# ygtxr1997/MSML

Measured on AMD Instinct MI355X. Metric: images/sec (112x112) ires50-MSML+PartialFC training step, higher is better.
Workload: dtype bf16; 1 GPU; iresnet50-MSML (OSB r18 + FM x4) + 85742-id ArcFace PartialFC, 112x112, batch 256/GPU, fwd+bwd+clip+SGD; global_batch=256, parallelism=dp1+class-parallel head, launch=eager, weight gradients + OSB on side streams

## Files before the change

### include/msml_hip.h

```cpp
#ifndef MSML_HIP_H
#define MSML_HIP_H

#include <stddef.h>
#include <stdint.h>

#ifdef __cplusplus
extern "C" {
#endif

#define MSML_ABI_VERSION 1

enum { MSML_F32 = 0, MSML_BF16 = 1, MSML_BF16X3 = 2,
       MSML_F64 = 3 };

enum {
  MSML_OK = 0,
  MSML_ERR_SHAPE = -1,
  MSML_ERR_DTYPE = -2,
  MSML_ERR_LAUNCH = -3,
  MSML_ERR_UNSUPPORTED = -4,
  MSML_ERR_WORKSPACE = -5,
  MSML_ERR_CAPACITY = -6
};

// ... 216 lines not shown

int msml_deconv4_bwd_data(const void* dy, const void* wp0, const void* wp1, void* dx0, void* dx1, int N, int H,
                          void* stream);

int msml_conv2d_bnbwd_rows(int coutp, int N, int P, int Q);
int msml_conv2d_bnbwd(const void* in0, int c0p, const void* wp, int kop, void* out, int coutp,
                      int N, int H, int W, int P, int Q, int R, int S, int stride, int pad_h,
                      int pad_w, int transposed, const void* bn_x, const float* bn_scale,
                      const float* bn_shift, const float* bn_alpha, const float* bn_mean,
                      const float* bn_invstd, float* partial, int rows_cap, int* rows_used,
                      void* stream);
int msml_bn_act_bwd_apply(const void* dy, const void* x, const float* scale, const float* shift,
                          const float* alpha, const float* save_mean, const float* save_invstd,
                          const float* partial, int rows, const void* add, void* dx,
                          float* dgamma, float* dbeta, float* dalpha, int accumulate, long M,
                          int C, float* coef_ws, int dtype, void* stream);

int msml_bn_act_bwd_apply_s2(const void* dy, const void* x, const float* scale, const float* shift,
                             const float* alpha, const float* save_mean, const float* save_invstd,
                             const float* partial, int rows, const void* add, int H, int W, void* dx,
                             float* dgamma, float* dbeta, float* dalpha, int accumulate, long M,
                             int C, float* coef_ws, int dtype, void* stream);
int msml_bn_act_bwd_apply_next_s2(const void* dy, const void* x, const float* scale,
                                  const float* shift, const float* alpha, const float* save_mean,
                                  const float* save_invstd, const float* partial, int rows,
                                  const void* add, int H, int W, void* dx, float* dgamma, float* dbeta,
                                  float* dalpha, int accumulate, long M, int C, float* coef_ws,
                                  const void* next_x, const float* next_mean,
                                  const float* next_invstd, float* next_partial, int dtype,
                                  void* stream);

int msml_conv2d_bnin_applies(int c0p, int coutp, int N, int H, int W, int P, int Q, int R, int S,
                             int stride, int pad_h, int pad_w, int want_stats);
int msml_conv2d_bnin(const void* in0, int c0p, const float* in_scale, const float* in_shift,
                     const float* in_alpha, const void* wp, int kop, void* out, int coutp,
                     float* stats, int N, int H, int W, int P, int Q, int R, int S, int stride,
                     int pad_h, int pad_w, void* stream);
int msml_conv_wgrad_bnin_applies(int up, int vp, int A, int Breal, int N, int H, int W, int P, int Q,
                                 int R, int S, int stride, int pad_h, int pad_w);
int msml_conv_wgrad_bnin(const void* u, int up, const void* v, int vp, const float* x_scale,
                         const float* x_shift, const float* x_alpha, float* dw, int A, int Breal,
                         int Btot, int boff, int N, int H, int W, int P, int Q, int R, int S,
                         int stride, int pad_h, int pad_w, int accumulate, void* workspace,
                         long ws_bytes, void* stream);

#define MSML_KERNEL_MFM 2
const char* msml_conv2d_kernel(int c0p, int c1p, int coutp, int N, int H, int W, int P, int Q,
                               int R, int S, int stride, int pad_h, int pad_w, int transposed,
                               int in_dtype, int out_dtype, int want_stats);

int msml_stem_im2col(const float* x, void* out, int N, int C, int H, int W, int P, int Q, int R,
                     int S, int stride, int pad, int KP, int dtype, void* stream);

int msml_stem_bwd_data(const void* dy, const float* w, float* dx, int N, int C, int H, int W, int P, int Q,
                       int Cout, int ldy, int R, int S, int stride, int pad, int dtype, void* stream);
int msml_stem_bwd_data_band(int C, int H, int W, int Cout, int R, int stride);

int msml_bn_act_bwd_apply_rows(long M, int C);
int msml_bn_act_bwd_apply_next(const void* dy, const void* x, const float* scale, const float* shift,
                               const float* alpha, const float* save_mean, const float* save_invstd,
                               const float* partial, int rows, const void* add, void* dx,
                               float* dgamma, float* dbeta, float* dalpha, int accumulate, long M,
                               int C, float* coef_ws, const void* next_x, const float* next_mean,
                               const float* next_invstd, float* next_partial, int dtype, void* stream);

int msml_conv2d_bnin_acc_applies(int c0p, int coutp, int N, int H, int W, int P, int Q, int R, int S, int stride,
                                 int pad_h, int pad_w);
int msml_conv2d_bnin_acc(const void* in0, int c0p, const double* acc_in, double count, const float* gamma,
                         const float* beta, float* running_mean, float* running_var, float momentum, float eps,
                         float* coef_out, const float* in_alpha, void* act_out, const void* wp, int kop, void* out,
                         int coutp, double* acc_out, int N, int H, int W, int P, int Q, int R, int S, int stride,
                         int pad_h, int pad_w, void* stream);

int msml_iblock_fwd_tables(int* nptr, int* nint, int* nflt);
int msml_iblock_fwd(const void* const* ptrs, const int* ints, const float* flts, void* stream);

int msml_probe_mfma(const void* seed, float* out, int wgs, int iters, void* stream);
int msml_probe_mfma_lds(const void* seed, float* out, int wgs, int iters, void* stream);


int msml_conv2d_mfm(const void* in0, int c0p, const void* wp, int kop, const float* bias, void* out, int coutp,
                    const void* residual, unsigned char* sel, int N, int H, int W, int P, int Q, int R, int S,
                    int stride, int pad_h, int pad_w, int dtype, void* stream);

int msml_mfm_bwd(const void* dy, const unsigned char* sel, void* dz, long M, int cp, int C, int czp, int dtype,
                 void* stream);

int msml_pool2_fwd(const void* x, void* y, int N, int H, int W, int cp, int dtype, void* stream);

int msml_pool2_bwd(const void* dy, const void* x, void* dx, int N, int H, int W, int cp, int dtype, void* stream);

int msml_template_pool(const float* feats, long n_rows, long ld, int E, int flip, const float* faceness,
                       const int* order, const int* media_start, const int* tmpl_media_start, const int* launch,
                       int n_templates, double* out, void* stream);
int msml_template_pair_score(const double* tn, int n_templates, int E, const int* r1, const int* r2, long n_pairs,
                             double* score, void* stream);
int msml_roc_blocks(int n);
int msml_roc_block_counts(const double* sorted, const unsigned char* label, int n, int* blk, void* stream);
int msml_roc_points(const double* sorted, const unsigned char* label, int n, const int* off, int* tps, int* fps,
                    void* stream);
int msml_roc_reduce_blocks(int n_points);
int msml_roc_reduce(const int* tps, const int* fps, int n_points, const double* target, int n_targets,
                    unsigned char* keep, unsigned long long* part, void* stream);
int msml_pair_cosdist(const float* emb, int n_pairs, int E, double* dist, void* stream);
int msml_pair_cosdist_f64(const double* emb, int n_pairs, int E, double* dist, void* stream);
int msml_rank_count(const double* sorted, int n, const double* q, int m, int strict, int* out, void* stream);
// ... 94 lines not shown
```

### msml_amd/csrc/conv_wgrad.hip

```cpp
#include <stdlib.h>

#include "common.h"
#include "conv_call.h"
#include "options.h"
#include "wgrad_call.h"

typedef __attribute__((ext_vector_type(4))) short s16x4;
typedef __attribute__((ext_vector_type(8))) short s16x8;

struct WgradArgs {
  const void* u; int up;
  const void* v; int vp;
  int N, H, W, P, Q, R, S, stride, pad_h, pad_w;
  float* ws;
  int arows;
  long Mpix;
  int chunk;
  float rcp_pq, rcp_q;
};

__device__ __forceinline__ void divmod(int m, int d, float rcp, int& q, int& r) {
  q = (int)((float)m * rcp);
  r = m - q * d;
  if (r < 0) { r += d; q--; }
// ... 212 lines not shown

#define WR_MAXTAPS 49
__global__ void __launch_bounds__(256) k_wgrad_reduce_rows(const float* __restrict__ ws, const DwPtrs dsts,
                                                           int splits, int arows, int taps, int vp, int A,
                                                           int Breal, int Btot, int boff, int accumulate) {
  __shared__ float tile[WR_MAXTAPS * 65];
  const long slab = (long)arows * taps * vp;
  ws += (long)blockIdx.y * splits * slab;
  float* __restrict__ dst = dsts.p[blockIdx.y];
  const int lane = threadIdx.x & 63, wave = threadIdx.x >> 6;
  const int bblocks = (vp + 63) >> 6;
  const int a = blockIdx.x / bblocks, b0 = (blockIdx.x - a * bblocks) << 6;
  const int b = b0 + lane;
  for (int tap = wave; tap < taps; tap += 4) {
    float acc[8];
#pragma unroll
    for (int k = 0; k < 8; k++) acc[k] = 0.f;
    if (b < vp) {
      const float* p = ws + ((long)a * taps + tap) * vp + b;
      int sp = 0;
      for (; sp + 8 <= splits; sp += 8) {
        float v[8];
#pragma unroll
        for (int k = 0; k < 8; k++) v[k] = p[(long)(sp + k) * slab];
#pragma unroll
        for (int k = 0; k < 8; k++) acc[k] += v[k];
      }
#pragma unroll
      for (int k = 0; k < 8; k++)
        if (sp + k < splits) acc[k] += p[(long)(sp + k) * slab];
    }
    tile[tap * 65 + lane] = ((acc[0] + acc[4]) + (acc[1] + acc[5])) + ((acc[2] + acc[6]) + (acc[3] + acc[7]));
  }
  __syncthreads();
  const int nb = Breal - b0 < 64 ? Breal - b0 : 64;
  float* out = dst + ((long)a * Btot + boff + b0) * taps;
  for (int j = threadIdx.x; j < nb * taps; j += 256) {
    const int bl = j / taps, tap = j - bl * taps;
    const float sum = tile[tap * 65 + bl];
    out[j] = accumulate ? out[j] + sum : sum;
  }
}

static void wgrad_reduce_launch_group(const float* ws, float* const* dw, int group, int splits, int up, int taps, int vp,
                                      int A, int Breal, int Btot, int boff, int accumulate, hipStream_t st) {
  DwPtrs d;
  for (int i = 0; i < WGRAD_MAXGROUP; i++) d.p[i] = dw[i < group ? i : 0];
  const int rowblocks = A * ((vp + 63) / 64);
  if (rowblocks >= 512 && taps > 1 && taps <= WR_MAXTAPS)
    k_wgrad_reduce_rows<<<dim3(rowblocks, group), 256, 0, st>>>(ws, d, splits, up, taps, vp, A, Breal, Btot, boff, accumulate);
  else
    k_wgrad_reduce<<<dim3(rowblocks * taps, group), 256, 0, st>>>(ws, d, splits, up, taps, vp, A, Breal, Btot, boff,
                                                                 accumulate);
}

static int wgrad_ntw(int vp, int taps) {
  const bool off = msml_opt().wgrad_no_multitap;
  const int wide = msml_opt().wgrad_multitap_wide;
  if (off || taps < 3) return 1;
  if (vp <= 64) return 3;
  return (wide && vp % 64 == 0 && vp <= wide) ? 3 : 1;
}

static int pick_tile(int c) { return c > 64 ? 128 : 64; }

static int pick_splits(long mpix, int out_tiles) {
  const long forced = msml_opt().wgrad_wgs;
  const long minchunk = msml_opt().wgrad_minchunk;
  long target = 1024;
  if (out_tiles <= 9 && mpix <= (1L << 20)) target = 512;
  else if (out_tiles > 48) target = 768;
  if (forced > 0) target = forced;
  long want = (target + out_tiles - 1) / out_tiles;
  long max_by_chunk = (mpix + minchunk - 1) / minchunk;
  long s = want < max_by_chunk ? want : max_by_chunk;
  if (s < 1) s = 1;
  if (s > WGRAD_MAXSPLITS) s = WGRAD_MAXSPLITS;
  return (int)s;
}

static void wgrad_tile_plan(const WgradShape& s, WgradPlan& p) {
  const int taps = s.R * s.S;
  const long mpix = (long)s.N * s.P * s.Q;
  p.ba = pick_tile(s.up);
  p.bb = pick_tile(s.vp);
  p.ntw = s.dtype == MSML_BF16 ? wgrad_ntw(s.vp, taps) : 1;
  const int tiles = p.ntw > 1 ? cdiv(s.up, p.ba) * cdiv(taps, p.ntw) * cdiv(s.vp, 64) : cdiv(s.up, p.ba) * cdiv(s.vp, p.bb) * taps;
  p.splits = pick_splits(mpix, tiles) / s.group;
  if (p.splits < 1) p.splits = 1;
  p.chunk = (int)(((mpix + p.splits - 1) / p.splits + 63) / 64 * 64);
}

static bool wgrad_fast_groupable(const WgradShape& s) { return s.R == 3 && s.S == 3 && s.stride == 1; }

static WgradPlan wgrad_plan(const WgradShape& s) {
  WgradPlan p;
  const bool bf16 = s.dtype == MSML_BF16, one = s.group == 1 && !s.bnin;
  if (bf16 && one && msml_wgrad_fc_applies(s)) {
    p.family = WGRAD_FC;
    p.splits = p.direct = 1;
  } else if (bf16 && one && (p.splits = msml_wgrad_n32_applies(s)) > 0) {
    p.family = WGRAD_N32;
  } else if (bf16 && one && (p.splits = msml_wgrad_line_applies(s)) > 0) {
    p.family = WGRAD_LINE;
  } else if (bf16 && (p.splits = msml_wgrad_halo_applies(s)) > 0) {
    p.family = WGRAD_HALO;
// ... 226 lines not shown
```

### msml_amd/csrc/wgrad_call.h

```cpp
#pragma once
#include "common.h"

#define WGRAD_MAXGROUP 8
#define WGRAD_MAXSPLITS 512

struct WgradShape {
  int up = 0, vp = 0;
  int A = 0, Breal = 0, Btot = 0, boff = 0;
  int N = 0, H = 0, W = 0, P = 0, Q = 0, R = 0, S = 0, stride = 1, pad_h = 0, pad_w = 0;
  int dtype = MSML_BF16;
  int group = 1;
  int bnin = 0;
  int dw_aligned = 1;
};

struct WgradCall : WgradShape {
  const void* const* u = nullptr;
  const void* const* v = nullptr;
  float* const* dw = nullptr;
  int accumulate = 0;
  float* ws = nullptr;
  long ws_bytes = 0;
  hipStream_t st = nullptr;
  const BnIn* xin = nullptr;
};

enum WgradFamily { WGRAD_NONE = 0, WGRAD_FC, WGRAD_N32, WGRAD_LINE, WGRAD_HALO, WGRAD_FAST, WGRAD_GENERIC };
enum { WGRAD_HALO_64 = 64, WGRAD_HALO_128 = 128, WGRAD_HALO_PAIR7 = 7 };

struct WgradPlan {
  int family = WGRAD_NONE;
  int variant = 0;
  int ba = 0, bb = 0, ntw = 0;
  int splits = 0;
  int chunk = 0;
  int direct = 0;
  long slab_bytes = 0;
  const char* refused = nullptr;
};

bool msml_wgrad_fc_applies(const WgradShape& s);
int msml_wgrad_n32_applies(const WgradShape& s);
int msml_wgrad_n32_max_splits(const WgradShape& s);
int msml_wgrad_line_applies(const WgradShape& s);
int msml_wgrad_line_max_splits(const WgradShape& s);
int msml_wgrad_halo_applies(const WgradShape& s);
int msml_wgrad_halo_variant(const WgradShape& s);
int msml_wgrad_halo_max_splits(const WgradShape& s);
bool msml_wgrad_fast_applies(const WgradShape& s);

void msml_wgrad_fc_launch(const WgradCall& c, const WgradPlan& p);
void msml_wgrad_n32_launch(const WgradCall& c, const WgradPlan& p);
void msml_wgrad_line_launch(const WgradCall& c, const WgradPlan& p);
void msml_wgrad_halo_launch(const WgradCall& c, const WgradPlan& p);
void msml_wgrad_fast_launch(const WgradCall& c, const WgradPlan& p);
```

### msml_amd/functional.py

```python
import os
import torch

from . import _lib, ops
from ._lib import BF16, DTYPE_OF, F32, TORCH_DTYPE, call
from .ops import cpad


class _ToNHWC(torch.autograd.Function):

    @staticmethod
    def forward(ctx, x, dtype):
        ctx.c, ctx.xdtype = x.shape[1], x.dtype
        return ops.to_nhwc(x.float(), dtype)

    @staticmethod
    def backward(ctx, g):
        dx = ops.to_nchw(g.contiguous(), ctx.c)
        return (dx if ctx.xdtype is torch.float32 else dx.to(ctx.xdtype)), None


def to_nhwc(x, dtype):
    return _ToNHWC.apply(x, dtype)


# ... 691 lines not shown
    stride, (ph, pw) = conv_m.stride[0], conv_m.padding
    coutp = cpad(cout)
    assert coutp == cout == bn_m.num_features
    wp = ops.PACKS.get(conv_m.weight, False, 0, cout, 0, cin, c0, c1, BF16)
    coef = _eval_bn_coef(bn_m, coutp)
    p = ops.conv_out_size(h, r, stride, ph, False)
    q = ops.conv_out_size(w, s, stride, pw, False)
    c1p = 0 if x1 is None else x1.shape[3]
    out = torch.empty(n, p, q, coutp, dtype=torch.bfloat16, device=x0.device)
    name = "conv_fused"
    if ops.PROFILE.on:
        name = ops.conv_label("N+bn", c0p, c1p, coutp, n, h, w, p, q, r, s, stride, ph, pw, 0, BF16, BF16, False)
    with ops.PROFILE.rec(name, 2.0 * n * p * q * cin * cout * r * s):
        call("msml_conv2d_fused", x0, c0p, x1, c1p, wp, wp.shape[0], coef[0], coef[1],
             prelu.weight if prelu is not None else None, residual, int(res_first), out, coutp,
             n, h, w, p, q, r, s, stride, ph, pw, 0)
    return out


class RawImage:

    def __init__(self, x, x3=False):
        self.raw = x
        self.dtype = torch.bfloat16
        self.x3 = x3
        self._nhwc = None

    def nhwc(self):
        if self._nhwc is None:
            self._nhwc = to_nhwc(self.raw, BF16)
        return self._nhwc

    def record_stream(self, stream):
        self.raw.record_stream(stream)


def _stem_pack(conv_m):
    w = conv_m.weight
    stamp = (w._version, ops.WEIGHT_EPOCH, w.data_ptr())
    hit = getattr(conv_m, "_msml_stem_pack", None)
    if hit is None or hit[0] != stamp:
        cout, cin, r, s = w.shape
        w2 = w.detach().permute(0, 2, 3, 1).reshape(cout, r * s * cin, 1, 1).contiguous()
        hit = (stamp, ops.pack_weight(w2, False, r * s * cin, 0, BF16))
        conv_m._msml_stem_pack = hit
    return hit[1]


class _StemConv(torch.autograd.Function):

    @staticmethod
    def forward(ctx, weight, conv_m, raw):
        cout, cin, r, s = weight.shape
        col = ops.stem_im2col(raw, r, s, conv_m.stride[0], conv_m.padding[0])
        ctx.xshape, ctx.geom = tuple(raw.shape), (conv_m.stride[0], conv_m.padding[0])
        wp = _stem_pack(conv_m)
        y, stats = ops.conv2d(col, None, wp, None, cpad(cout), 1, 1, 1, 0, 0, False, want_stats=True,
                              real=(r * s * cin, cout))
        ctx.set_materialize_grads(False)
        ctx.wparam = weight
        ctx.save_for_backward(col)
        ctx.mark_non_differentiable(stats)
        return y, stats

    @staticmethod
    def backward(ctx, dy, _dstats):
        if dy is None:
            return None, None, None
        (col,) = ctx.saved_tensors
        w = ctx.wparam
        cout, cin, r, s = w.shape
        k = r * s * cin
        dw2 = torch.empty(cout, k, 1, 1, dtype=torch.float32, device=dy.device)
        dy = dy.contiguous()
        ops.conv_wgrad(dy, col, dw2, cout, k, k, 0, 1, 1, 1, 0, 0)
        dw = dw2.view(cout, r, s, cin).permute(0, 3, 1, 2)
        dx = None
        if ctx.needs_input_grad[2]:
            n, _, h, wd = ctx.xshape
            dx = ops.stem_bwd_data(dy, w, n, cin, h, wd, r, s, ctx.geom[0], ctx.geom[1])
        if ops.inplace(w):
            w.grad.view(w.shape).add_(dw)
            ops.grad_ready(w)
            return None, None, dx
        return dw.contiguous(), None, dx


def stem_conv_bn(raw, conv_m, bn_m, prelu):
    if raw.x3:
        return stem_conv_bn_x3(raw, conv_m, bn_m, prelu)
    if not bn_m.training and not torch.is_grad_enabled():
        cout, cin, r, s = conv_m.weight.shape
        col = ops.stem_im2col(raw.raw, r, s, conv_m.stride[0], conv_m.padding[0])
        wp = _stem_pack(conv_m)
        coef = _eval_bn_coef(bn_m, cpad(cout))
        n, p, q, kp = col.shape
        out = torch.empty(n, p, q, cpad(cout), dtype=torch.bfloat16, device=col.device)
        name = "conv_fused"
        if ops.PROFILE.on:
            name = ops.conv_label("N+bn", kp, 0, cpad(cout), n, p, q, p, q, 1, 1, 1, 0, 0, 0, BF16, BF16, False)
        with ops.PROFILE.rec(name, 2.0 * n * p * q * r * s * cin * cout):
            call("msml_conv2d_fused", col, kp, None, 0, wp, wp.shape[0], coef[0], coef[1],
                 prelu.weight if prelu is not None else None, None, 0, out, cpad(cout), n, p, q, p, q, 1, 1,
                 1, 0, 0, 0)
        return out
    y, stats = _StemConv.apply(conv_m.weight, conv_m, raw.raw)
    return bn_act(y, stats if stats.numel() else None, bn_m, prelu, emit_stats=True)


class SplitT:
    __slots__ = ("t", "c")
    dtype = "bf16x3"

    def __init__(self, t, c):
        self.t, self.c = t, c

    @property
    def shape(self):
        n, h, w, _ = self.t.shape
        return (n, h, w, self.c)

    @property
    def device(self):
        return self.t.device

    def detach(self):
        return self

# ... 505 lines not shown
```

### msml_amd/ops.py

```python
import ctypes
import os
import weakref

import torch

from . import _lib
from ._lib import BF16, DTYPE_OF, F32, TORCH_DTYPE, call, try_call


class _Profile:

    def __init__(self):
        self.on = False
        self.recs = []
        self.by_size = bool(os.environ.get("MSML_PROFILE_BY_SIZE"))

    def start(self):
        self.recs = []
        self.on = True

    def rec(self, name, flops=0.0, nbytes=0.0):
        if not self.on:
            return _NO_REC
        if nbytes and not flops and self.by_size:
# ... 121 lines not shown
            ent = [torch.zeros(max(self.CHUNK, n), dtype=torch.float64, device=device), 0, cap]
            self.chunks[key] = ent
        out = ent[0][ent[1]:ent[1] + n].view(ACC_ROWS, nq, c)
        ent[1] += n
        return out


ACC_ARENA = _AccArena()


def acc_applies(c, dtype):
    return ACC_STATS and dtype == BF16 and c % 8 == 0 and 256 % (c // 8) == 0


def stats_acc(c, device, nq=2):
    return ACC_ARENA.get(c, device, nq)


def rows4(t):
    assert t.dtype is torch.float32
    p = t.data_ptr()
    s = t.stride(0) * 4
    return (p, p + s, p + s + s, p + 3 * s)


_UNIT_COEF = {}


def unit_coef(cp, device):
    key = (cp, device)
    u = _UNIT_COEF.get(key)
    if u is None:
        if torch.cuda.is_current_stream_capturing():
            return (torch.ones(cp, dtype=torch.float32, device=device), torch.zeros(cp, dtype=torch.float32, device=device))
        u = _UNIT_COEF[key] = (torch.ones(cp, dtype=torch.float32).to(device), torch.zeros(cp, dtype=torch.float32).to(device))
        torch.cuda.current_stream(device).synchronize()
    return u


def conv_out_size(h, r, stride, pad, transposed, out_pad=0):
    if transposed:
        return (h - 1) * stride - 2 * pad + r + out_pad
    return (h + 2 * pad - r) // stride + 1


def stem_im2col(x, r, s, stride, pad, kp=32, dtype=BF16):
    n, c, h, w = x.shape
    p = conv_out_size(h, r, stride, pad, False)
    q = conv_out_size(w, s, stride, pad, False)
    out = torch.empty(n, p, q, kp, dtype=TORCH_DTYPE[dtype], device=x.device)
    with PROFILE.rec("stem_im2col", 0.0, x.numel() * 4 + out.numel() * out.element_size()):
        call("msml_stem_im2col", x.contiguous(), out, n, c, h, w, p, q, r, s, stride, pad, kp, dtype)
    return out


NO_STEM_BWD_DATA = os.environ.get("MSML_NO_STEM_BWD_DATA") is not None


def stem_bwd_data(dy, weight, n, c, h, w, r, s, stride, pad):
    if NO_STEM_BWD_DATA:
        raise RuntimeError("msml_amd: the input image requires a gradient, and MSML_NO_STEM_BWD_DATA switches "
                           "msml_stem_bwd_data off; there is no other path for it")
    p = conv_out_size(h, r, stride, pad, False)
    q = conv_out_size(w, s, stride, pad, False)
    cout = weight.shape[0]
    assert dy.is_contiguous() and tuple(dy.shape[:3]) == (n, p, q) and tuple(weight.shape) == (cout, c, r, s)
    wd = weight.detach().float().contiguous()
    dx = torch.empty(n, c, h, w, dtype=torch.float32, device=dy.device)
    with PROFILE.rec("stem_bwd_data", 0.0, dy.numel() * dy.element_size() + dx.numel() * 4):
        call("msml_stem_bwd_data", dy, wd, dx, n, c, h, w, p, q, cout, dy.shape[3], r, s, stride, pad, DTYPE_OF[dy.dtype])
    return dx


def conv_label(kind, c0p, c1p, coutp, n, h, w, p, q, r, s, stride, pad_h, pad_w, transposed, in_dtype, out_dtype,
               want_stats):
    kern = _lib.value("msml_conv2d_kernel", c0p, c1p, coutp, n, h, w, p, q, r, s, stride, pad_h, pad_w,
                      int(transposed), in_dtype, out_dtype, int(bool(want_stats))).decode()
    return "conv %s c%d+%d->%d %dx%d k%dx%d s%d n%d [%s]" % (kind, c0p, c1p, coutp, h, w, r, s, stride, n, kern)


def conv2d(x0, x1, wp, bias, coutp, r, s, stride, pad_h, pad_w, transposed, p=None, q=None,
           out_dtype=None, want_stats=False, real=None):
    n, h, w, c0p = x0.shape
    c1p = x1.shape[3] if x1 is not None else 0
    if p is None:
        p = conv_out_size(h, r, stride, pad_h, transposed)
        q = conv_out_size(w, s, stride, pad_w, transposed)
    in_dtype = DTYPE_OF[x0.dtype]
    out_dtype = in_dtype if out_dtype is None else out_dtype
    out = torch.empty(n, p, q, coutp, dtype=TORCH_DTYPE[out_dtype], device=x0.device)
    stats = None
    acc = want_stats and out_dtype == BF16 and acc_applies(coutp, in_dtype)
    if acc:
        stats = stats_acc(coutp, x0.device)
    elif want_stats:
        tiles = (n * p * q + tile_m(coutp) - 1) // tile_m(coutp)
        stats = torch.empty(tiles, 2, coutp, dtype=torch.float32, device=x0.device)
    cin, cout = real if real is not None else (c0p + c1p, coutp)
    pix = n * h * w if transposed else n * p * q
    name = "conv_igemm"
    if PROFILE.on:
        name = conv_label("T" if transposed else "N", c0p, c1p, coutp, n, h, w, p, q, r, s, stride, pad_h, pad_w,
                          transposed, in_dtype, out_dtype, want_stats)
    with PROFILE.rec(name, 2.0 * pix * cin * cout * r * s):
        call("msml_conv2d_acc" if acc else "msml_conv2d", x0, c0p, x1, c1p, wp, wp.shape[0], bias, out, coutp, stats,
             n, h, w, p, q, r, s, stride, pad_h, pad_w, int(transposed), in_dtype, out_dtype)
# ... 402 lines not shown
```

Measured before the change: 9028 images/sec.

## Fuse stem im2col into direct MFMA stem conv and stem wgrad kernels

```diff
diff --git a/include/msml_hip.h b/include/msml_hip.h
--- a/include/msml_hip.h
+++ b/include/msml_hip.h
@@ -292,6 +292,17 @@
 int msml_stem_im2col(const float* x, void* out, int N, int C, int H, int W, int P, int Q, int R,
                      int S, int stride, int pad, int KP, int dtype, void* stream);
 
+int msml_stem_conv_applies(int C, int H, int W, int R, int S, int stride, int pad, int coutp, int dtype);
+int msml_stem_conv_rows(int P);
+int msml_stem_conv(const float* x, const void* wp, int kop, int ktot, const float* bias, void* out, int coutp,
+                   void* stats, int stats_acc, int N, int C, int H, int W, int P, int Q, int R, int S, int stride,
+                   int pad, int dtype, void* stream);
+int msml_stem_wgrad_splits(int N, int C, int H, int W, int R, int S, int stride, int pad, int up, int dtype);
+int msml_stem_wgrad_rows(void);
+int msml_stem_wgrad(const void* dy, int up, const float* x, float* dw, int A, int N, int C, int H, int W, int P,
+                    int Q, int R, int S, int stride, int pad, int accumulate, void* workspace, long ws_bytes, int dtype,
+                    void* stream);
+
 int msml_stem_bwd_data(const void* dy, const float* w, float* dx, int N, int C, int H, int W, int P, int Q,
                        int Cout, int ldy, int R, int S, int stride, int pad, int dtype, void* stream);
 int msml_stem_bwd_data_band(int C, int H, int W, int Cout, int R, int stride);
diff --git a/msml_amd/csrc/conv_wgrad.hip b/msml_amd/csrc/conv_wgrad.hip
--- a/msml_amd/csrc/conv_wgrad.hip
+++ b/msml_amd/csrc/conv_wgrad.hip
@@ -288,6 +288,11 @@
   else
     k_wgrad_reduce<<<dim3(rowblocks * taps, group), 256, 0, st>>>(ws, d, splits, up, taps, vp, A, Breal, Btot, boff,
                                                                  accumulate);
+}
+
+void msml_wgrad_reduce_launch(const WgradCall& c, const WgradPlan& p) {
+  wgrad_reduce_launch_group(c.ws, c.dw, c.group, p.splits, c.up, c.R * c.S, c.vp, c.A, c.Breal, c.Btot, c.boff, c.accumulate,
+                            c.st);
 }
 
 static int wgrad_ntw(int vp, int taps) {
diff --git a/msml_amd/csrc/stem.hip b/msml_amd/csrc/stem.hip
--- /dev/null
+++ b/msml_amd/csrc/stem.hip
@@ -0,0 +1,450 @@
+#include <stdlib.h>
+
+#include "common.h"
+#include "options.h"
+#include "wgrad_call.h"
+
+typedef __attribute__((ext_vector_type(4))) short s16x4;
+typedef __attribute__((ext_vector_type(8))) short s16x8;
+
+#define ST_WMAX 128
+#define ST_WP (ST_WMAX + 2)
+
+template <int NR>
+__device__ __forceinline__ int stem_koff(int k) {
+  const int tap = k / 3, c = k - tap * 3, r = tap / 3, s = tap - r * 3;
+  return tap < 9 ? (c * NR + r) * ST_WP + s : -1;
+}
+
+struct StemConvArgs {
+  const float* x;
+  const unsigned short* wp;
+  unsigned short* out;
+  const float* bias;
+  float* stats;
+  int stats_acc;
+  int N, H, W, P, Q, ktot;
+};
+
+#define STEM_CONV_ROWS 16
+
+template <typename T, int STRIDE, int NCOW>
+__global__ void __launch_bounds__(256) k_stem_conv(const StemConvArgs p) {
+#if defined(__HIP_DEVICE_COMPILE__)
+  static_assert(sizeof(T) == 2, "bf16 storage only");
+  constexpr int ROWS = STEM_CONV_ROWS, NR = (ROWS - 1) * STRIDE + 3, COUT = 32 * NCOW;
+  constexpr int C8W = COUT / 8, OPB = COUT * 2, NOJ = 32 * C8W / 64, ZERO = 3 * NR * ST_WP;
+  __shared__ unsigned short tile[3 * NR * ST_WP + 8];
+  __shared__ __attribute__((aligned(16))) char xout_all[4 * 32 * OPB];
+  __shared__ __attribute__((aligned(16))) float btab[COUT];
+  __shared__ float red[4 * 2 * COUT];
+  const int t = threadIdx.x, lane = t & 63;
+  const int wave = __builtin_amdgcn_readfirstlane(t >> 6);
+  const int r32 = lane & 31, h = lane >> 5;
+  const int tiles_y = (p.P + ROWS - 1) / ROWS;
+  const int n = blockIdx.x / tiles_y, oy0 = (blockIdx.x - n * tiles_y) * ROWS;
+  const int nrows = p.P - oy0 < ROWS ? p.P - oy0 : ROWS, npix = nrows * p.Q;
+  const int W = p.W;
+
+  {
+    constexpr int IMG_PT = (3 * NR * ST_WMAX + 255) / 256;
+    const float* xn = p.x + (long)n * 3 * p.H * W;
+    const int iy0 = oy0 * STRIDE - 1;
+    float ir[IMG_PT];
+#pragma unroll
+    for (int k = 0; k < IMG_PT; k++) {
+      const int i = t + 256 * k, ix = i & (ST_WMAX - 1), cr = i >> 7 < 3 * NR ? i >> 7 : 3 * NR - 1, c = cr / NR, row = cr - c * NR;
+      const int iy = iy0 + row, iyc = iy < 0 ? 0 : (iy < p.H ? iy : p.H - 1), ixc = ix < W ? ix : W - 1;
+      const float v = xn[((long)c * p.H + iyc) * W + ixc];
+      ir[k] = ((unsigned)iy < (unsigned)p.H) ? v : 0.f;
+    }
+#pragma unroll
+    for (int k = 0; k < IMG_PT; k++) {
+      const int i = t + 256 * k, ix = i & (ST_WMAX - 1), cr = i >> 7;
+      if (cr < 3 * NR && ix < W) tile[cr * ST_WP + ix + 1] = f2bf(ir[k]);
+    }
+    for (int i = t; i < 3 * NR * 2; i += 256) tile[(i >> 1) * ST_WP + ((i & 1) ? W + 1 : 0)] = 0;
+    if (t < 8) tile[ZERO + t] = 0;
+    if (t < COUT) btab[t] = p.bias ? p.bias[t] : 0.f;
+  }
+  u32x4 wf[NCOW][2];
+#pragma unroll
+  for (int i = 0; i < NCOW; i++)
+#pragma unroll
+    for (int kk = 0; kk < 2; kk++)
+      wf[i][kk] = *reinterpret_cast<const u32x4*>(p.wp + (long)(32 * i + r32) * p.ktot + (kk * 2 + h) * 8);
+  int koff[2][8];
+#pragma unroll
+  for (int kk = 0; kk < 2; kk++)
+#pragma unroll
+    for (int j = 0; j < 8; j++) koff[kk][j] = stem_koff<NR>(kk * 16 + h * 8 + j);
+
+  char* xout = xout_all + wave * (32 * OPB);
+  auto okey = [](int row) -> int { return C8W == 4 ? ((row >> 2) & 3) : (row & 7); };
+  const int opl = lane / C8W;
+  const int cl = (lane % C8W) ^ okey(opl);
+  f32x4 s1[4 * NCOW], s2[4 * NCOW];
+#pragma unroll
+  for (int g = 0; g < 4 * NCOW; g++) s1[g] = s2[g] = f32x4{0.f, 0.f, 0.f, 0.f};
+  unsigned short* const outp = p.out + ((long)n * p.P + oy0) * p.Q * COUT;
+  __syncthreads();
+
+  const int nunits = (npix + 31) >> 5, upw = (nunits + 3) >> 2;
+  for (int u = wave * upw; u < nunits && u < (wave + 1) * upw; u++) {
+    const int pl = u * 32 + r32;
+    const bool valid = pl < npix;
+    const int pc = valid ? pl : 0;
+    const int orow = pc / p.Q, ox = pc - orow * p.Q;
+    const int base = orow * STRIDE * ST_WP + ox * STRIDE;
+    u32x4 xb[2];
+#pragma unroll
+    for (int kk = 0; kk < 2; kk++)
+#pragma unroll
+      for (int e = 0; e < 4; e++) {
+        const int o0 = koff[kk][2 * e], o1 = koff[kk][2 * e + 1];
+        const unsigned int lo = tile[o0 < 0 ? ZERO : base + o0], hi = tile[o1 < 0 ? ZERO : base + o1];
+        xb[kk][e] = lo | (hi << 16);
+      }
+    f32x16 acc[NCOW];
+#pragma unroll
+    for (int i = 0; i < NCOW; i++)
+#pragma unroll
+      for (int e = 0; e < 16; e++) acc[i][e] = 0.f;
+#pragma unroll
+    for (int kk = 0; kk < 2; kk++)
+#pragma unroll
+      for (int i = 0; i < NCOW; i++)
+        acc[i] = __builtin_amdgcn_mfma_f32_32x32x16_bf16(__builtin_bit_cast(bf16x8, wf[i][kk]), __builtin_bit_cast(bf16x8, xb[kk]),
+                                                         acc[i], 0, 0, 0);
+#pragma unroll
+    for (int i = 0; i < NCOW; i++) {
+      u32x2 pk[4];
+#pragma unroll
+      for (int g = 0; g < 4; g++) {
+        const f32x4 bv = *reinterpret_cast<const f32x4*>(btab + 32 * i + 8 * g + 4 * h);
+        float v[4];
+#pragma unroll
+        for (int j = 0; j < 4; j++) {
+          v[j] = acc[i][g * 4 + j] + bv[j];
+          if (valid) {
+            s1[4 * i + g][j] += v[j];
+            s2[4 * i + g][j] += v[j] * v[j];
+          }
+        }
+        pk[g][0] = (unsigned int)f2bf(v[0]) | ((unsigned int)f2bf(v[1]) << 16);
+        pk[g][1] = (unsigned int)f2bf(v[2]) | ((unsigned int)f2bf(v[3]) << 16);
+      }
+      u32x4 ch[2];
+#pragma unroll
+      for (int e = 0; e < 2; e++) {
+        auto r01 = __builtin_amdgcn_permlane32_swap(pk[0][e], pk[1][e], false, false);
+        auto r23 = __builtin_amdgcn_permlane32_swap(pk[2][e], pk[3][e], false, false);
+        ch[0][e] = r01[0]; ch[0][2 + e] = r01[1];
+        ch[1][e] = r23[0]; ch[1][2 + e] = r23[1];
+      }
+#pragma unroll
+      for (int c = 0; c < 2; c++)
+        *reinterpret_cast<u32x4*>(xout + r32 * OPB + (((4 * i + 2 * c + h) ^ okey(r32)) << 4)) = ch[c];
+    }
+    __builtin_amdgcn_wave_barrier();
+#pragma unroll
+    for (int j = 0; j < NOJ; j++) {
+      const int m = u * 32 + j * (64 / C8W) + opl;
+      const u32x4 v = *reinterpret_cast<const u32x4*>(xout + (j * 64 + lane) * 16);
+      if (m < npix) *reinterpret_cast<u32x4*>(outp + (long)m * COUT + cl * 8) = v;
+    }
+    __builtin_amdgcn_wave_barrier();
+  }
+
+  if (p.stats) {
+#pragma unroll
+    for (int g = 0; g < 4 * NCOW; g++)
+#pragma unroll
+      for (int j = 0; j < 4; j++) {
+        const float a = wave_half_sum(s1[g][j]), b = wave_half_sum(s2[g][j]);
+        if (r32 == 0) {
+          red[(wave * 2 + 0) * COUT + 8 * g + 4 * h + j] = a;
+          red[(wave * 2 + 1) * COUT + 8 * g + 4 * h + j] = b;
+        }
+      }
+    __syncthreads();
+    for (int e = t; e < 2 * COUT; e += 256) {
+      const int q = e / COUT, c = e - q * COUT;
+      float sum = 0.f;
+#pragma unroll
+      for (int w = 0; w < 4; w++) sum += red[(w * 2 + q) * COUT + c];
+      stats_emit(p.stats, p.stats_acc, blockIdx.x, q, COUT, c, sum);
+    }
+  }
+#endif
+}
+
+static bool stem_geometry_ok(int C, int H, int W, int R, int S, int stride, int pad, int coutp, int dtype) {
+  return C == 3 && R == 3 && S == 3 && pad == 1 && (stride == 1 || stride == 2) && H > 0 && W > 0 && W <= ST_WMAX &&
+         (coutp == 32 || coutp == 64) && dtype == MSML_BF16;
+}
+
+extern "C" int msml_stem_conv_applies(int C, int H, int W, int R, int S, int stride, int pad, int coutp, int dtype) {
+  return stem_geometry_ok(C, H, W, R, S, stride, pad, coutp, dtype) ? 1 : 0;
+}
+
+extern "C" int msml_stem_conv_rows(int P) { return cdiv(P, STEM_CONV_ROWS); }
+
+extern "C" int msml_stem_conv(const float* x, const void* wp, int kop, int ktot, const float* bias, void* out, int coutp,
+                              void* stats, int stats_acc, int N, int C, int H, int W, int P, int Q, int R, int S,
+                              int stride, int pad, int dtype, void* stream) {
+  MSML_CHECK(x && wp && out, MSML_ERR_SHAPE, "stem_conv: null pointer");
+  MSML_CHECK(N > 0 && H > 0 && W > 0 && P > 0 && Q > 0, MSML_ERR_SHAPE, "stem_conv: bad dims");
+  MSML_CHECK(dtype == MSML_BF16 || dtype == MSML_F32, MSML_ERR_DTYPE, "stem_conv: unsupported dtype %d", dtype);
+  MSML_CHECK(stem_geometry_ok(C, H, W, R, S, stride, pad, coutp, dtype), MSML_ERR_UNSUPPORTED,
+             "stem_conv: serves 3 channels, 3x3, pad 1, stride 1 or 2, W <= %d, 32 or 64 stored output channels, bf16", ST_WMAX);
+  MSML_CHECK(P == (H - 1) / stride + 1 && Q == (W - 1) / stride + 1, MSML_ERR_SHAPE, "stem_conv: P x Q is not the conv's output size");
+  MSML_CHECK(kop >= coutp && ktot >= 32 && ktot % 8 == 0, MSML_ERR_SHAPE, "stem_conv: packed weight [%d][%d] too small", kop, ktot);
+  MSML_CHECK((size_t)wp % 16 == 0 && (size_t)out % 16 == 0 && (size_t)x % 4 == 0 && (!bias || (size_t)bias % 4 == 0) &&
+                 (!stats || (size_t)stats % (stats_acc ? 8 : 4) == 0),
+             MSML_ERR_SHAPE, "stem_conv: misaligned pointer");
+  StemConvArgs a{x, (const unsigned short*)wp, (unsigned short*)out, bias, (float*)stats, stats_acc ? 1 : 0, N, H, W, P, Q, ktot};
+  const dim3 grid((unsigned)((long)N * cdiv(P, STEM_CONV_ROWS)));
+  hipStream_t st = (hipStream_t)stream;
+  if (stride == 1) {
+    if (coutp == 32) k_stem_conv<unsigned short, 1, 1><<<grid, 256, 0, st>>>(a);
+    else k_stem_conv<unsigned short, 1, 2><<<grid, 256, 0, st>>>(a);
+  } else {
+    if (coutp == 32) k_stem_conv<unsigned short, 2, 1><<<grid, 256, 0, st>>>(a);
+    else k_stem_conv<unsigned short, 2, 2><<<grid, 256, 0, st>>>(a);
+  }
+  MSML_LAUNCH_OK("stem_conv");
+  return MSML_OK;
+}
+
+struct StemWgradArgs {
+  const float* x;
+  const unsigned short* dy;
+  float* ws;
+  int N, H, W, P, Q, tiles_y, ntiles, chunk;
+};
+
+#define STEM_WGRAD_ROWS 2
+
+template <typename T, int STRIDE, int NUP>
+__global__ void __launch_bounds__(256) k_stem_wgrad(const StemWgradArgs p) {
+#if defined(__HIP_DEVICE_COMPILE__)
+  static_assert(sizeof(T) == 2, "bf16 storage only");
+  constexpr int RB = STEM_WGRAD_ROWS, NR = (RB - 1) * STRIDE + 3, UP = 32 * NUP, C8 = UP / 8, ZERO = 3 * NR * ST_WP;
+  constexpr int NBLK = RB * ST_WMAX / 16, HB = NBLK * 1024;
+  constexpr int DY_PT = NBLK * 16 * C8 / 256, IMG_PT = (3 * NR * ST_WMAX + 255) / 256;
+  __shared__ __attribute__((aligned(16))) char dyb[NUP * HB];
+  __shared__ __attribute__((aligned(16))) char pscr_all[4 * 1024];
+  __shared__ unsigned short tile[3 * NR * ST_WP + 8];
+  static_assert(NUP * HB >= NUP * 16 * 64 * 4, "the end-of-kernel sums fit the dY region");
+  const int t = threadIdx.x, lane = t & 63;
+  const int wave = __builtin_amdgcn_readfirstlane(t >> 6);
+  const int W = p.W, Q = p.Q;
+  const int t_begin = blockIdx.x * p.chunk;
+  int t_end = t_begin + p.chunk;
+  if (t_end > p.ntiles) t_end = p.ntiles;
+
+  for (int i = t; i < 3 * NR * 2; i += 256) tile[(i >> 1) * ST_WP + ((i & 1) ? W + 1 : 0)] = 0;
+  if (t < 8) tile[ZERO + t] = 0;
+
+  struct Regs {
+    u32x4 dr[DY_PT];
+    float ir[IMG_PT];
+  };
+  auto tile_pix = [&](int tl, int& n, int& oy0) -> int {
+    n = tl / p.tiles_y;
+    oy0 = (tl - n * p.tiles_y) * RB;
+    return (p.P - oy0 < RB ? p.P - oy0 : RB) * Q;
+  };
+  auto load_tile = [&](int tl, Regs& r) {
+    int n, oy0;
+    const int npix = tile_pix(tl, n, oy0);
+    const unsigned short* src = p.dy + ((long)n * p.P + oy0) * Q * UP;
+#pragma unroll
+    for (int k = 0; k < DY_PT; k++) {
+      const int i = t + 256 * k;
+      const bool ok = i < npix * C8;
+      r.dr[k] = *reinterpret_cast<const u32x4*>(src + (long)(ok ? i : 0) * 8);
+    }
+    const float* xn = p.x + (long)n * 3 * p.H * W;
+    const int iy0 = oy0 * STRIDE - 1;
+#pragma unroll
+    for (int k = 0; k < IMG_PT; k++) {
+      const int i = t + 256 * k, ix = i & (ST_WMAX - 1), cr = i >> 7 < 3 * NR ? i >> 7 : 3 * NR - 1, c = cr / NR, row = cr - c * NR;
+      const int iy = iy0 + row, iyc = iy < 0 ? 0 : (iy < p.H ? iy : p.H - 1), ixc = ix < W ? ix : W - 1;
+      r.ir[k] = xn[((long)c * p.H + iyc) * W + ixc];
+    }
+  };
+  auto store_tile = [&](int tl, const Regs& r) {
+    int n, oy0;
+    const int npix = tile_pix(tl, n, oy0);
+    const int iy0 = oy0 * STRIDE - 1;
+#pragma unroll
+    for (int k = 0; k < DY_PT; k++) {
+      const int i = t + 256 * k, px = i / C8, c = i - px * C8;
+      *reinterpret_cast<u32x4*>(dyb + (c >> 2) * HB + (px >> 4) * 1024 + (px & 15) * 64 + (c & 3) * 16) =
+          px < npix ? r.dr[k] : u32x4{0, 0, 0, 0};
+    }
+#pragma unroll
+    for (int k = 0; k < IMG_PT; k++) {
+      const int i = t + 256 * k, ix = i & (ST_WMAX - 1), cr = i >> 7, c = cr / NR, row = cr - c * NR;
+      if (cr < 3 * NR && ix < W) tile[cr * ST_WP + ix + 1] = ((unsigned)(iy0 + row) < (unsigned)p.H) ? f2bf(r.ir[k]) : (unsigned short)0;
+    }
+  };
+
+  f32x16 acc[NUP];
+#pragma unroll
+  for (int i = 0; i < NUP; i++)
+#pragma unroll
+    for (int e = 0; e < 16; e++) acc[i][e] = 0.f;
+  const int g4 = lane >> 4, i16 = lane & 15, q4 = i16 >> 2, pp = i16 & 3;
+  const int aofs = (8 * (g4 >> 1) + q4) * 64 + (2 * (g4 & 1) + (pp >> 1)) * 16 + (pp & 1) * 8;
+  typedef __attribute__((address_space(3))) s16x4* tr_ptr;
+  auto tr2 = [&](const char* lo) -> s16x8 {
+    s16x4 l = __builtin_amdgcn_ds_read_tr16_b64_v4i16((tr_ptr)(lo));
+    s16x4 hh = __builtin_amdgcn_ds_read_tr16_b64_v4i16((tr_ptr)(lo + 256));
+    s16x8 o;
+    o[0] = l[0]; o[1] = l[1]; o[2] = l[2]; o[3] = l[3];
+    o[4] = hh[0]; o[5] = hh[1]; o[6] = hh[2]; o[7] = hh[3];
+    return o;
+  };
+  char* pscr = pscr_all + wave * 1024;
+  const int ppx = lane >> 2, pkc = lane & 3;
+  int koff[8];
+#pragma unroll
+  for (int j = 0; j < 8; j++) koff[j] = stem_koff<NR>(pkc * 8 + j);
+
+  auto ksteps = [&](int tl) {
+    int n_, oy_;
+    const int npix = tile_pix(tl, n_, oy_);
+    const int nblk = (npix + 15) >> 4;
+    for (int j = wave; j < nblk; j += 4) {
+      const int pl = j * 16 + ppx, pc = pl < npix ? pl : 0;
+      const int orow = pc / Q, ox = pc - orow * Q;
+      const int base = orow * STRIDE * ST_WP + ox * STRIDE;
+      u32x4 v;
+#pragma unroll
+      for (int e = 0; e < 4; e++) {
+        const int o0 = koff[2 * e], o1 = koff[2 * e + 1];
+        const unsigned int lo = tile[o0 < 0 ? ZERO : base + o0], hi = tile[o1 < 0 ? ZERO : base + o1];
+        v[e] = lo | (hi << 16);
+      }
+      *reinterpret_cast<u32x4*>(pscr + ppx * 64 + pkc * 16) = v;
+      __builtin_amdgcn_wave_barrier();
+      const s16x8 fb = tr2(pscr + aofs);
+#pragma unroll
+      for (int i = 0; i < NUP; i++) {
+        const s16x8 fa = tr2(dyb + i * HB + j * 1024 + aofs);
+        acc[i] = __builtin_amdgcn_mfma_f32_32x32x16_bf16(__builtin_bit_cast(bf16x8, fa), __builtin_bit_cast(bf16x8, fb), acc[i],
+                                                         0, 0, 0);
+      }
+      __builtin_amdgcn_wave_barrier();
+    }
+  };
+  Regs r;
+  int tl = t_begin;
+  if (tl < t_end) load_tile(tl, r);
+  for (; tl < t_end; tl++) {
+    __syncthreads();
+    store_tile(tl, r);
+    __syncthreads();
+    if (tl + 1 < t_end) load_tile(tl + 1, r);
+    ksteps(tl);
+  }
+
+  float* red = reinterpret_cast<float*>(dyb);
+  const int h = lane >> 5, b = lane & 31;
+  for (int w = 0; w < 4; w++) {
+    __syncthreads();
+    if (wave == w) {
+#pragma unroll
+      for (int i = 0; i < NUP; i++)
+#pragma unroll
+        for (int e = 0; e < 16; e++) {
+          const int idx = (i * 16 + e) * 64 + lane;
+          if (w == 0) red[idx] = acc[i][e];
+          else if (w < 3) red[idx] += acc[i][e];
+          else {
+            const int a = 32 * i + (e & 3) + 8 * (e >> 2) + 4 * h;
+            p.ws[((long)blockIdx.x * UP + a) * 32 + b] = red[idx] + acc[i][e];
+          }
+        }
+    }
+  }
+#endif
+}
+
+int msml_stem_wgrad_applies(const WgradShape& s) {
+  if (!stem_geometry_ok(3, s.H, s.W, s.R, s.S, s.stride, s.pad_h, s.up, s.dtype) || s.pad_w != 1 || s.vp != 32 || s.Breal != 27 ||
+      s.group != 1 || s.bnin)
+    return 0;
+  if (s.N <= 0 || s.P != (s.H - 1) / s.stride + 1 || s.Q != (s.W - 1) / s.stride + 1) return 0;
+  const long ntiles = (long)s.N * cdiv(s.P, STEM_WGRAD_ROWS);
+  if (ntiles >= (1L << 30)) return 0;
+  const long forced = msml_opt().wgrad_wgs, minchunk = msml_opt().wgrad_minchunk;
+  long splits = forced > 0 ? forced : 2L * msml_num_cus();
+  const long mpix = (long)s.N * s.P * s.Q, by_chunk = (mpix + minchunk - 1) / (minchunk > 0 ? minchunk : 1);
+  if (splits > by_chunk) splits = by_chunk;
+  if (splits > ntiles) splits = ntiles;
+  if (splits > WGRAD_MAXSPLITS) splits = WGRAD_MAXSPLITS;
+  if (splits < 1) splits = 1;
+  const long chunk = (ntiles + splits - 1) / splits;
+  return (int)((ntiles + chunk - 1) / chunk);
+}
+
+static WgradShape stem_wgrad_shape(int N, int C, int H, int W, int R, int S, int stride, int pad, int up, int A, int dtype) {
+  WgradShape s;
+  s.up = up; s.vp = 32; s.A = A; s.Breal = (C == 3 && R == 3 && S == 3) ? 27 : 0; s.Btot = s.Breal; s.boff = 0;
+  s.N = N; s.H = H; s.W = W; s.R = R; s.S = S; s.stride = stride; s.pad_h = s.pad_w = pad; s.dtype = dtype;
+  s.P = stride > 0 ? (H + 2 * pad - R) / stride + 1 : 0;
+  s.Q = stride > 0 ? (W + 2 * pad - S) / stride + 1 : 0;
+  return s;
+}
+
+extern "C" int msml_stem_wgrad_splits(int N, int C, int H, int W, int R, int S, int stride, int pad, int up, int dtype) {
+  return msml_stem_wgrad_applies(stem_wgrad_shape(N, C, H, W, R, S, stride, pad, up, up, dtype));
+}
+extern "C" int msml_stem_wgrad_rows() { return STEM_WGRAD_ROWS; }
+
+extern "C" int msml_stem_wgrad(const void* dy, int up, const float* x, float* dw, int A, int N, int C, int H, int W, int P,
+                               int Q, int R, int S, int stride, int pad, int accumulate, void* workspace, long ws_bytes,
+                               int dtype, void* stream) {
+  MSML_CHECK(dy && x && dw && workspace, MSML_ERR_SHAPE, "stem_wgrad: null pointer");
+  MSML_CHECK(N > 0 && H > 0 && W > 0 && P > 0 && Q > 0 && A > 0 && A <= up, MSML_ERR_SHAPE, "stem_wgrad: bad dims");
+  MSML_CHECK(dtype == MSML_BF16 || dtype == MSML_F32, MSML_ERR_DTYPE, "stem_wgrad: unsupported dtype %d", dtype);
+  MSML_CHECK((size_t)dy % 16 == 0 && (size_t)x % 4 == 0 && (size_t)dw % 4 == 0 && (size_t)workspace % 16 == 0, MSML_ERR_SHAPE,
+             "stem_wgrad: misaligned pointer");
+  WgradShape s = stem_wgrad_shape(N, C, H, W, R, S, stride, pad, up, A, dtype);
+  MSML_CHECK(stem_geometry_ok(C, H, W, R, S, stride, pad, up, dtype), MSML_ERR_UNSUPPORTED,
+             "stem_wgrad: serves 3 channels, 3x3, pad 1, stride 1 or 2, W <= %d, 32 or 64 stored dY channels, bf16", ST_WMAX);
+  MSML_CHECK(P == s.P && Q == s.Q, MSML_ERR_SHAPE, "stem_wgrad: P x Q is not the conv's output size");
+  const int splits = msml_stem_wgrad_applies(s);
+  MSML_CHECK(splits > 0, MSML_ERR_UNSUPPORTED, "stem_wgrad: shape not covered");
+  const long need = (long)splits * up * 32 * (long)sizeof(float);
+  MSML_CHECK(ws_bytes >= need, MSML_ERR_WORKSPACE, "stem_wgrad: workspace %ld < %ld bytes", ws_bytes, need);
+  StemWgradArgs a;
+  a.x = x; a.dy = (const unsigned short*)dy; a.ws = (float*)workspace;
+  a.N = N; a.H = H; a.W = W; a.P = P; a.Q = Q;
+  a.tiles_y = cdiv(P, STEM_WGRAD_ROWS);
+  a.ntiles = N * a.tiles_y;
+  a.chunk = cdiv(a.ntiles, splits);
+  hipStream_t st = (hipStream_t)stream;
+  if (stride == 1) {
+    if (up == 32) k_stem_wgrad<unsigned short, 1, 1><<<splits, 256, 0, st>>>(a);
+    else k_stem_wgrad<unsigned short, 1, 2><<<splits, 256, 0, st>>>(a);
+  } else {
+    if (up == 32) k_stem_wgrad<unsigned short, 2, 1><<<splits, 256, 0, st>>>(a);
+    else k_stem_wgrad<unsigned short, 2, 2><<<splits, 256, 0, st>>>(a);
+  }
+  MSML_LAUNCH_OK("stem_wgrad");
+  WgradCall c;
+  static_cast<WgradShape&>(c) = s;
+  c.R = c.S = 1; c.H = P; c.W = Q; c.stride = 1; c.pad_h = c.pad_w = 0;
+  float* dwp = dw;
+  c.dw = &dwp; c.accumulate = accumulate; c.ws = (float*)workspace; c.ws_bytes = ws_bytes; c.st = st;
+  WgradPlan pl;
+  pl.splits = splits;
+  msml_wgrad_reduce_launch(c, pl);
+  MSML_LAUNCH_OK("stem_wgrad_reduce");
+  return MSML_OK;
+}
diff --git a/msml_amd/csrc/wgrad_call.h b/msml_amd/csrc/wgrad_call.h
--- a/msml_amd/csrc/wgrad_call.h
+++ b/msml_amd/csrc/wgrad_call.h
@@ -54,3 +54,6 @@
 void msml_wgrad_line_launch(const WgradCall& c, const WgradPlan& p);
 void msml_wgrad_halo_launch(const WgradCall& c, const WgradPlan& p);
 void msml_wgrad_fast_launch(const WgradCall& c, const WgradPlan& p);
+
+int msml_stem_wgrad_applies(const WgradShape& s);
+void msml_wgrad_reduce_launch(const WgradCall& c, const WgradPlan& p);
diff --git a/msml_amd/functional.py b/msml_amd/functional.py
--- a/msml_amd/functional.py
+++ b/msml_amd/functional.py
@@ -767,14 +767,19 @@
     @staticmethod
     def forward(ctx, weight, conv_m, raw):
         cout, cin, r, s = weight.shape
-        col = ops.stem_im2col(raw, r, s, conv_m.stride[0], conv_m.padding[0])
         ctx.xshape, ctx.geom = tuple(raw.shape), (conv_m.stride[0], conv_m.padding[0])
         wp = _stem_pack(conv_m)
-        y, stats = ops.conv2d(col, None, wp, None, cpad(cout), 1, 1, 1, 0, 0, False, want_stats=True,
-                              real=(r * s * cin, cout))
+        ctx.fused = ops.stem_fused_applies(raw, weight, *ctx.geom)
+        if ctx.fused:
+            y, stats = ops.stem_conv(raw, wp, None, cout, ctx.geom[0], ctx.geom[1], want_stats=True)
+            ctx.save_for_backward(raw)
+        else:
+            col = ops.stem_im2col(raw, r, s, conv_m.stride[0], conv_m.padding[0])
+            y, stats = ops.conv2d(col, None, wp, None, cpad(cout), 1, 1, 1, 0, 0, False, want_stats=True,
+                                  real=(r * s * cin, cout))
+            ctx.save_for_backward(col)
         ctx.set_materialize_grads(False)
         ctx.wparam = weight
-        ctx.save_for_backward(col)
         ctx.mark_non_differentiable(stats)
         return y, stats
 
@@ -788,7 +793,10 @@
         k = r * s * cin
         dw2 = torch.empty(cout, k, 1, 1, dtype=torch.float32, device=dy.device)
         dy = dy.contiguous()
-        ops.conv_wgrad(dy, col, dw2, cout, k, k, 0, 1, 1, 1, 0, 0)
+        if ctx.fused:
+            ops.stem_wgrad(dy, col, dw2, cout, ctx.geom[0], ctx.geom[1])
+        else:
+            ops.conv_wgrad(dy, col, dw2, cout, k, k, 0, 1, 1, 1, 0, 0)
         dw = dw2.view(cout, r, s, cin).permute(0, 3, 1, 2)
         dx = None
         if ctx.needs_input_grad[2]:
diff --git a/msml_amd/ops.py b/msml_amd/ops.py
--- a/msml_amd/ops.py
+++ b/msml_amd/ops.py
@@ -197,6 +197,48 @@
     with PROFILE.rec("stem_im2col", 0.0, x.numel() * 4 + out.numel() * out.element_size()):
         call("msml_stem_im2col", x.contiguous(), out, n, c, h, w, p, q, r, s, stride, pad, kp, dtype)
     return out
+
+
+NO_STEM_FUSED = os.environ.get("MSML_NO_STEM_FUSED") is not None
+
+
+def stem_fused_applies(x, weight, stride, pad):
+    if NO_STEM_FUSED:
+        return False
+    cout, c, r, s = weight.shape
+    _, _, h, w = x.shape
+    coutp = cpad(cout)
+    return bool(_lib.value("msml_stem_conv_applies", c, h, w, r, s, stride, pad, coutp, BF16) and
+                _lib.value("msml_stem_wgrad_splits", x.shape[0], c, h, w, r, s, stride, pad, coutp, BF16))
+
+
+def stem_conv(x, wp, bias, cout, stride, pad, want_stats=False):
+    n, c, h, w = x.shape
+    coutp = cpad(cout)
+    p = conv_out_size(h, 3, stride, pad, False)
+    q = conv_out_size(w, 3, stride, pad, False)
+    out = torch.empty(n, p, q, coutp, dtype=torch.bfloat16, device=x.device)
+    stats, acc = None, False
+    if want_stats:
+        acc = acc_applies(coutp, BF16)
+        if acc:
+            stats = stats_acc(coutp, x.device)
+        else:
+            stats = torch.empty(n * _lib.value("msml_stem_conv_rows", p), 2, coutp, dtype=torch.float32, device=x.device)
+    with PROFILE.rec("stem_conv", 2.0 * n * p * q * 9 * c * cout):
+        call("msml_stem_conv", x.contiguous(), wp, wp.shape[0], wp.shape[1], bias, out, coutp, stats, int(acc), n, c, h, w,
+             p, q, 3, 3, stride, pad, BF16)
+    return out, stats
+
+
+def stem_wgrad(dy, x, dw, cout, stride, pad, accumulate=False):
+    n, c, h, w = x.shape
+    _, p, q, up = dy.shape
+    ws = workspace(wgrad_ws_need(up, 32, n, p, q, 1, 1), dy.device, "wgrad")
+    with PROFILE.rec("stem_wgrad", 2.0 * n * p * q * cout * 9 * c):
+        call("msml_stem_wgrad", dy, up, x.contiguous(), dw, cout, n, c, h, w, p, q, 3, 3, stride, pad, int(accumulate), ws,
+             ws.numel(), BF16)
+    return dw
 
 
 NO_STEM_BWD_DATA = os.environ.get("MSML_NO_STEM_BWD_DATA") is not None
```

Measured after the change: 9080 images/sec (median of 6 runs). Within noise of the previous version (+0.6%).
